# zkp-gravity/0g-halo2

Hardware: AMD Instinct MI355X
Metric: create_proof proofs/hour, model_28input_256entry_1hash_1bpi (higher is better)
Workload: dtype u32x8 (254-bit Montgomery integers)

## Files before the change

### 0g-halo2_amd/csrc/field.h

```cpp
#pragma once

#include <hip/hip_runtime.h>
#include <stdint.h>

#define ZG_HD __host__ __device__ __forceinline__

namespace zg {

struct alignas(16) Fe {
    uint32_t l[8];
};

struct FrParams {
    static ZG_HD uint32_t p(int i) {
        constexpr uint32_t P[8] = {0xf0000001u, 0x43e1f593u, 0x79b97091u, 0x2833e848u,
                                   0x8181585du, 0xb85045b6u, 0xe131a029u, 0x30644e72u};
        return P[i];
    }
    static constexpr uint32_t P_TOP = 0x30644e72u;
    static constexpr uint32_t INV = 0xefffffffu;
    static constexpr bool IS_FR = true;
    static ZG_HD Fe one() {
        return Fe{{0x4ffffffbu, 0xac96341cu, 0x9f60cd29u, 0x36fc7695u, 0x7879462eu, 0x666ea36fu,
                   0x9a07df2fu, 0x0e0a77c1u}};
// ... 122 lines not shown
    static ZG_HD Fe dbl(const Fe& a) { return add(a, a); }

    static ZG_HD Fe mul(const Fe& a, const Fe& b) {
#if defined(__HIP_DEVICE_COMPILE__)
        uint64_t acc = 0;
        uint32_t ovf = 0;
        uint32_t m[8], r[8];
#include "mont_mul_gfx950.inc"
        Fe o;
#pragma unroll
        for (int i = 0; i < 8; i++) o.l[i] = r[i];
        reduce_once(o);
        return o;
#else
        typedef unsigned __int128 u128;
        uint64_t A[4], B[4], M[4], t[6] = {0, 0, 0, 0, 0, 0};
        for (int i = 0; i < 4; i++) {
            A[i] = (uint64_t)a.l[2 * i] | ((uint64_t)a.l[2 * i + 1] << 32);
            B[i] = (uint64_t)b.l[2 * i] | ((uint64_t)b.l[2 * i + 1] << 32);
            M[i] = (uint64_t)P::p(2 * i) | ((uint64_t)P::p(2 * i + 1) << 32);
        }
        const uint64_t ninv32 = P::INV;
        const uint64_t inv64 = ninv32 * (2 + M[0] * ninv32);
        for (int i = 0; i < 4; i++) {
            u128 c = 0;
            for (int j = 0; j < 4; j++) {
                c += (u128)A[j] * B[i] + t[j];
                t[j] = (uint64_t)c;
                c >>= 64;
            }
            c += t[4];
            t[4] = (uint64_t)c;
            t[5] = (uint64_t)(c >> 64);
            const uint64_t m = t[0] * inv64;
            c = (u128)m * M[0] + t[0];
            c >>= 64;
            for (int j = 1; j < 4; j++) {
                c += (u128)m * M[j] + t[j];
                t[j - 1] = (uint64_t)c;
                c >>= 64;
            }
            c += t[4];
            t[3] = (uint64_t)c;
            t[4] = t[5] + (uint64_t)(c >> 64);
        }
        Fe o;
        for (int i = 0; i < 4; i++) {
            o.l[2 * i] = (uint32_t)t[i];
            o.l[2 * i + 1] = (uint32_t)(t[i] >> 32);
        }
        reduce_once(o);
        return o;
#endif
    }

    static ZG_HD Fe sqr(const Fe& a) { return mul(a, a); }

    static ZG_HD Fe from_raw(const Fe& a) { return mul(a, P::r2()); }

    static ZG_HD Fe to_raw(const Fe& a) {
        Fe one_raw = fe_zero();
        one_raw.l[0] = 1;
        return mul(a, one_raw);
    }

    static ZG_HD Fe from_u64(uint64_t v) {
        Fe t = fe_zero();
        t.l[0] = (uint32_t)v;
        t.l[1] = (uint32_t)(v >> 32);
        return from_raw(t);
    }

    static ZG_HD Fe pow(const Fe& a, const uint32_t e[8]) {
        Fe res = one();
        for (int i = 7; i >= 0; i--)
            for (int b = 31; b >= 0; b--) {
                res = sqr(res);
                if ((e[i] >> b) & 1) res = mul(res, a);
            }
        return res;
    }

    static ZG_HD Fe pow_u64(const Fe& a, uint64_t e) {
        Fe res = one();
        bool started = false;
        for (int b = 63; b >= 0; b--) {
            if (started) res = sqr(res);
            if ((e >> b) & 1) {
                res = mul(res, a);
                started = true;
            }
        }
        return res;
    }

    static ZG_HD Fe inv_fermat(const Fe& a) {
        uint32_t e[8];
#pragma unroll
        for (int i = 0; i < 8; i++) e[i] = P::p(i);
        e[0] -= 2;
        return pow(a, e);
    }

    static ZG_HD Fe inv(const Fe& a) {
        if (fe_is_zero(a)) return a;
#if !defined(__HIP_DEVICE_COMPILE__)
// ... 148 lines not shown
```

### 0g-halo2_amd/csrc/ntt.hip

```cpp
#include "poly.h"
#include "field9.h"

namespace zg {

struct NttArgs {
    const Fe* in;
    Fe* out;
    const Fe* tw;
    const Fe* tw_x;
    const Fe* tw_m;
    uint32_t tw_shift;
    size_t in_stride;
    size_t out_stride;
    uint32_t in_per, out_per;
    size_t in_outer, out_outer;
    uint32_t log_n, log_n1, log_n2;
    uint32_t in_len;
    uint32_t out_len;
    uint32_t coset_in;
    uint32_t coset_out;
    uint32_t scale_out;
    Fe zin0, zin1, zin2, zout0, zout1, zout2, scale;
};

__device__ __forceinline__ uint32_t bitrev(uint32_t v, uint32_t bits) {
    return bits == 0 ? 0u : (__brev(v) >> (32 - bits));
}

__device__ __forceinline__ Fe ld_fe(const Fe* p) {
    Fe r;
    const uint4* q = reinterpret_cast<const uint4*>(p);
    uint4 a = q[0], b = q[1];
    r.l[0] = a.x; r.l[1] = a.y; r.l[2] = a.z; r.l[3] = a.w;
    r.l[4] = b.x; r.l[5] = b.y; r.l[6] = b.z; r.l[7] = b.w;
    return r;
}

__device__ __forceinline__ void st_fe(Fe* p, const Fe& v) {
    uint4* q = reinterpret_cast<uint4*>(p);
    q[0] = make_uint4(v.l[0], v.l[1], v.l[2], v.l[3]);
    q[1] = make_uint4(v.l[4], v.l[5], v.l[6], v.l[7]);
}

template <int LOG_T, bool COLS, bool FIRST>
__global__ __launch_bounds__(1 << (LOG_T - 2)) void ntt_pass_kernel(NttArgs a) {
    constexpr uint32_t T = 1u << LOG_T;
    constexpr uint32_t NT = T / 4;
    extern __shared__ __align__(16) unsigned char smem[];
    uint4* XL = reinterpret_cast<uint4*>(smem);
    uint4* XH = XL + T;
    uint4* TL = XH + T;
    uint4* TH = TL + (1u << ((COLS ? a.log_n1 : a.log_n2) > 0 ? (COLS ? a.log_n1 : a.log_n2) - 1 : 0));
    auto slot = [](uint32_t i) { return i ^ ((i >> 3) & 7u) ^ ((i >> 6) & 7u) ^ ((i >> 9) & 7u); };
    auto ldx = [&](uint32_t i) {
        const uint32_t s = slot(i);
        const uint4 lo = XL[s], hi = XH[s];
        return Fe{{lo.x, lo.y, lo.z, lo.w, hi.x, hi.y, hi.z, hi.w}};
    };
    auto stx = [&](uint32_t i, const Fe& v) {
        const uint32_t s = slot(i);
        XL[s] = make_uint4(v.l[0], v.l[1], v.l[2], v.l[3]);
        XH[s] = make_uint4(v.l[4], v.l[5], v.l[6], v.l[7]);
    };
    auto ldt = [&](uint32_t i) {
        const uint32_t s = slot(i);
        const uint4 lo = TL[s], hi = TH[s];
        return Fe{{lo.x, lo.y, lo.z, lo.w, hi.x, hi.y, hi.z, hi.w}};
    };

    const uint32_t tid = threadIdx.x;
    const uint32_t log_m = COLS ? a.log_n1 : a.log_n2;
    const uint32_t M = 1u << log_m;
    const uint32_t N1 = 1u << a.log_n1, N2 = 1u << a.log_n2;
    uint32_t log_cnt = LOG_T - log_m;
    if (!COLS && log_cnt > a.log_n1) log_cnt = a.log_n1;
    const uint32_t cnt = 1u << log_cnt;
    const uint32_t tile = M << log_cnt;

    uint32_t nblk = gridDim.x, bid = blockIdx.x;
    if ((nblk & 7u) == 0) bid = (bid & 7u) * (nblk >> 3) + (bid >> 3);
    const uint32_t base = bid << log_cnt;

    const Fe* in = a.in + (size_t)(blockIdx.y / a.in_per) * a.in_outer + (size_t)(blockIdx.y % a.in_per) * a.in_stride;
    Fe* out = a.out + (size_t)(blockIdx.y / a.out_per) * a.out_outer + (size_t)(blockIdx.y % a.out_per) * a.out_stride;

    {
        const uint32_t tw_shift = a.log_n - log_m;
        for (uint32_t t = tid; t < M / 2; t += NT) {
            const Fe w = ld_fe(a.tw + ((size_t)t << tw_shift));
            const uint32_t s = slot(t);
            TL[s] = make_uint4(w.l[0], w.l[1], w.l[2], w.l[3]);
            TH[s] = make_uint4(w.l[4], w.l[5], w.l[6], w.l[7]);
        }
    }

    for (uint32_t e = tid; e < tile; e += NT) {
        uint32_t g, li;
        if (COLS) {
            uint32_t c = e & (cnt - 1), j1 = e >> log_cnt;
            g = j1 * N2 + base + c;
            li = e;
        } else {
            uint32_t j2 = e & (M - 1), r = e >> log_m;
            g = (base + r) * N2 + j2;
            li = e;
        }
        Fe v;
        if (FIRST) {
            if (g < a.in_len) {
                v = ld_fe(in + g);
                if (a.coset_in) {
                    const uint32_t m3 = g % 3u;
                    if (m3 != 0 || a.coset_in == 2) v = Fr::mul(v, m3 == 1 ? a.zin1 : m3 == 2 ? a.zin2 : a.zin0);
                }
            } else {
                v = fe_zero();
            }
        } else {
            v = ld_fe(in + g);
        }
        stx(li, v);
    }
    __syncthreads();

    auto at = [&](uint32_t sub, uint32_t e) { return COLS ? (e << log_cnt) + sub : (sub << log_m) + e; };
    uint32_t st = 0;
    if (FIRST && COLS && log_m >= 2) {
        const uint32_t nz_rows = (a.in_len + N2 - 1) >> a.log_n2;
        const uint32_t quarter = M >> 2, half = M >> 1;
        if (nz_rows <= quarter) {
            for (uint32_t g = tid; g < tile / 4; g += NT) {
                const uint32_t sub = g & (cnt - 1), i = g >> log_cnt;
                if (i >= nz_rows) continue;
                const uint32_t i0 = at(sub, i), i1 = at(sub, i + quarter), i2 = at(sub, i + half), i3 = at(sub, i + half + quarter);
                const Fe x0 = ldx(i0);
                Fe a2 = x0;
                if (i != 0) a2 = Fr::mul(x0, ldt(i));
                stx(i2, a2);
                if (i != 0) {
                    const Fe w = ldt(i << 1);
                    stx(i1, Fr::mul(x0, w));
                    stx(i3, Fr::mul(a2, w));
                } else {
                    stx(i1, x0);
                    stx(i3, a2);
                }
            }
            __syncthreads();
            st = 2;
        }
    }
    for (; st + 1 < log_m; st += 2) {
        const uint32_t log_half = log_m - st - 1, log_q = log_half - 1;
        const uint32_t half = 1u << log_half, quarter = 1u << log_q;
        for (uint32_t g = tid; g < tile / 4; g += NT) {
            uint32_t sub, b;
            if (COLS) {
                sub = g & (cnt - 1);
                b = g >> log_cnt;
            } else {
                b = g & (M / 4 - 1);
                sub = g >> (log_m - 2);
            }
            const uint32_t blk = b >> log_q, i = b & (quarter - 1);
            const uint32_t e0 = (blk << (log_half + 1)) + i;
            const uint32_t i0 = at(sub, e0), i1 = at(sub, e0 + quarter), i2 = at(sub, e0 + half), i3 = at(sub, e0 + half + quarter);
            const Fe x0 = ldx(i0), x1 = ldx(i1), x2 = ldx(i2), x3 = ldx(i3);
            const Fe a0 = Fr::add(x0, x2), a1 = Fr::add(x1, x3);
            Fe a2 = Fr::sub(x0, x2), a3 = Fr::sub(x1, x3);
            const uint32_t t0 = i << st;
            if (t0 != 0) a2 = Fr::mul(a2, ldt(t0));
            a3 = Fr::mul(a3, ldt((i + quarter) << st));
            const uint32_t t1 = i << (st + 1);
            stx(i0, Fr::add(a0, a1));
            stx(i2, Fr::add(a2, a3));
            Fe b1 = Fr::sub(a0, a1), b3 = Fr::sub(a2, a3);
            if (t1 != 0) {
                const Fe w = ldt(t1);
                b1 = Fr::mul(b1, w);
                b3 = Fr::mul(b3, w);
            }
            stx(i1, b1);
            stx(i3, b3);
        }
        __syncthreads();
    }
    const uint32_t nbf = tile / 2;
    for (; st < log_m; st++) {
        const uint32_t log_half = log_m - st - 1;
        const uint32_t half = 1u << log_half;
        for (uint32_t bf = tid; bf < nbf; bf += NT) {
            uint32_t s, b;
            if (COLS) {
                s = bf & (cnt - 1);
                b = bf >> log_cnt;
            } else {
                b = bf & (M / 2 - 1);
                s = bf >> (log_m - 1);
            }
            uint32_t blk = b >> log_half, i = b & (half - 1);
            uint32_t lo = (blk << (log_half + 1)) + i, hi = lo + half;
            uint32_t ilo = at(s, lo), ihi = at(s, hi);
            Fe u = ldx(ilo), v = ldx(ihi);
            stx(ilo, Fr::add(u, v));
            Fe d = Fr::sub(u, v);
            uint32_t twi = i << st;
            if (twi != 0) d = Fr::mul(d, ldt(twi));
            stx(ihi, d);
        }
        __syncthreads();
    }

    if (COLS) {
        for (uint32_t e = tid; e < tile; e += NT) {
            uint32_t c = e & (cnt - 1), pos = e >> log_cnt;
            uint32_t k1 = bitrev(pos, log_m);
            uint32_t j2 = base + c;
            Fe v = ldx(e);
            v = Fr::mul(v, ld_fe(a.tw_x + j2 * k1));
            st_fe(out + (size_t)k1 * N2 + j2, v);
        }
    } else {
        for (uint32_t e = tid; e < tile; e += NT) {
            uint32_t r = e & (cnt - 1), k2 = e >> log_cnt;
            uint32_t pos = bitrev(k2, log_m);
            uint32_t k = (base + r) + N1 * k2;
            if (k >= a.out_len) continue;
            Fe v = ldx((r << log_m) + pos);
            if (a.scale_out) v = Fr::mul(v, a.scale);
            if (a.coset_out) {
                const uint32_t m3 = k % 3u;
                if (m3 != 0 || a.coset_out == 2) v = Fr::mul(v, m3 == 1 ? a.zout1 : m3 == 2 ? a.zout2 : a.zout0);
            }
            st_fe(out + k, v);
        }
    }
}

template <int LOG_T, bool COLS, bool FIRST>
__global__ __launch_bounds__(1 << (LOG_T - 2)) void ntt9_pass_kernel(NttArgs a) {
    constexpr uint32_t T = 1u << LOG_T;
    constexpr uint32_t NT = T / 4;
    extern __shared__ __align__(16) unsigned char smem[];
    const uint32_t log_m = COLS ? a.log_n1 : a.log_n2;
    const uint32_t M = 1u << log_m;
    const uint32_t S = a.tw_shift;
    const uint32_t TWN = (M / 2) >> S ? (M / 2) >> S : 1;
    uint4* XL = reinterpret_cast<uint4*>(smem);
    uint4* XH = XL + T;
    uint4* TL = XH + T;
    uint4* TH = TL + TWN;
    int32_t* X8 = reinterpret_cast<int32_t*>(TH + TWN);
    int32_t* T8 = X8 + T;
    auto slot = [](uint32_t i) { return i ^ ((i >> 3) & 7u) ^ ((i >> 6) & 7u) ^ ((i >> 9) & 7u); };
    auto ld3 = [&](const uint4* L, const uint4* H, const int32_t* E, uint32_t i) {
        const uint32_t s = slot(i);
        const uint4 lo = L[s], hi = H[s];
        F9 r;
        r.l[0] = (int32_t)lo.x; r.l[1] = (int32_t)lo.y; r.l[2] = (int32_t)lo.z; r.l[3] = (int32_t)lo.w;
        r.l[4] = (int32_t)hi.x; r.l[5] = (int32_t)hi.y; r.l[6] = (int32_t)hi.z; r.l[7] = (int32_t)hi.w;
        r.l[8] = E[s];
        return r;
    };
    auto st3 = [&](uint4* L, uint4* H, int32_t* E, uint32_t i, const F9& v) {
        const uint32_t s = slot(i);
        L[s] = make_uint4((uint32_t)v.l[0], (uint32_t)v.l[1], (uint32_t)v.l[2], (uint32_t)v.l[3]);
        H[s] = make_uint4((uint32_t)v.l[4], (uint32_t)v.l[5], (uint32_t)v.l[6], (uint32_t)v.l[7]);
        E[s] = v.l[8];
    };
    auto ldx = [&](uint32_t i) { return ld3(XL, XH, X8, i); };
    auto stx = [&](uint32_t i, const F9& v) { st3(XL, XH, X8, i, v); };
    const Fe* twm9 = a.tw_m + M;
    auto ldt = [&](uint32_t i, uint32_t st) { return st >= S ? ld3(TL, TH, T8, i >> S) : f9_unpack(ld_fe(twm9 + i)); };

    const uint32_t tid = threadIdx.x;
    const uint32_t N1 = 1u << a.log_n1, N2 = 1u << a.log_n2;
    uint32_t log_cnt = LOG_T - log_m;
    if (!COLS && log_cnt > a.log_n1) log_cnt = a.log_n1;
    const uint32_t cnt = 1u << log_cnt;
    const uint32_t tile = M << log_cnt;

    uint32_t nblk = gridDim.x, bid = blockIdx.x;
    if ((nblk & 7u) == 0) bid = (bid & 7u) * (nblk >> 3) + (bid >> 3);
    const uint32_t base = bid << log_cnt;

    const Fe* in = a.in + (size_t)(blockIdx.y / a.in_per) * a.in_outer + (size_t)(blockIdx.y % a.in_per) * a.in_stride;
// ... 83 lines not shown
            if (reduce) s0 = Fr9::mul(s0, Fr9Params::one());
            stx(i0, s0);
            stx(i2, f9_norm(f9_add(a2, a3)));
            const F9 w = ldt(i << (st + 1), st + 1);
            stx(i1, Fr9::mul(f9_norm(f9_sub(a0, a1)), w));
            stx(i3, Fr9::mul(f9_sub(a2, a3), w));
        }
        __syncthreads();
    }
    const uint32_t nbf = tile / 2;
    for (; st < log_m; st++) {
        for (uint32_t bf = tid; bf < nbf; bf += NT) {
            uint32_t s, b;
            if (COLS) {
                s = bf & (cnt - 1);
                b = bf >> log_cnt;
            } else {
                b = bf & (M / 2 - 1);
                s = bf >> (log_m - 1);
            }
            const uint32_t ilo = at(s, b << 1), ihi = at(s, (b << 1) + 1);
            const F9 u = ldx(ilo), v = ldx(ihi);
            stx(ilo, f9_norm(f9_add(u, v)));
            stx(ihi, f9_norm(f9_sub(u, v)));
        }
        __syncthreads();
    }

    if (COLS) {
        for (uint32_t e = tid; e < tile; e += NT) {
            uint32_t c = e & (cnt - 1), pos = e >> log_cnt;
            uint32_t k1 = bitrev(pos, log_m);
            uint32_t j2 = base + c;
            const F9 v = Fr9::mul(ldx(e), f9_unpack(ld_fe(a.tw_x + j2 * k1)));
            st_fe(out + (size_t)k1 * N2 + j2, f9_reduce_pack<Fr9Params>(v));
        }
    } else {
        for (uint32_t e = tid; e < tile; e += NT) {
            uint32_t r = e & (cnt - 1), k2 = e >> log_cnt;
            uint32_t pos = bitrev(k2, log_m);
            uint32_t k = (base + r) + N1 * k2;
            if (k >= a.out_len) continue;
            F9 v = ldx((r << log_m) + pos);
            if (a.scale_out) v = Fr9::mul(v, f9_unpack(a.scale));
            if (a.coset_out) {
                const uint32_t m3 = k % 3u;
                if (m3 != 0 || a.coset_out == 2) v = Fr9::mul(v, f9_unpack(m3 == 1 ? a.zout1 : m3 == 2 ? a.zout2 : a.zout0));
            }
            st_fe(out + k, f9_reduce_pack<Fr9Params>(v));
        }
    }
}

__global__ void twiddle_kernel(Fe* tw, Fe omega, Fe s, uint32_t n) {
    constexpr uint32_t CH = 16;
    uint32_t i0 = (blockIdx.x * blockDim.x + threadIdx.x) * CH;
    if (i0 >= n) return;
    const Fe c261 = Fr9Params::c261_fe();
    Fe cur = Fr::mul(Fr::pow_u64(omega, i0), s);
    for (uint32_t j = 0; j < CH && i0 + j < n; j++) {
        st_fe(tw + i0 + j, cur);
        st_fe(tw + n + i0 + j, Fr::mul(cur, c261));
        cur = Fr::mul(cur, omega);
    }
}

constexpr uint32_t MAX_SCALED_TABLES = 8;
int get_twiddles(zg_ctx* ctx, uint32_t log_n, const Fe& omega, Fe** out, const Fe* scale) {
    const Fe s = scale ? *scale : Fr::one();
    TwiddleKey key;
    key.log_n = log_n;
    memcpy(key.omega.data(), &omega, 32);
    memcpy(key.scale.data(), &s, 32);
    DeviceState& ds = device_state(ctx->device);
    std::lock_guard<std::mutex> lock(ds.mu);
    auto it = ds.twiddles.find(key);
    if (it != ds.twiddles.end()) {
        *out = it->second;
        return ZG_OK;
    }
    if (scale) {
        const Fe one = Fr::one();
        uint32_t scaled = 0;
        for (const auto& kv : ds.twiddles) scaled += kv.first.log_n == log_n && memcmp(kv.first.scale.data(), &one, 32) != 0;
        if (scaled >= MAX_SCALED_TABLES) {
            *out = nullptr;
            return ZG_OK;
        }
    }
    uint32_t n = 1u << log_n;
    Fe* tw = nullptr;
    gate_yield(ctx);
    ZG_HIP(hipMalloc(&tw, (size_t)2 * n * sizeof(Fe)));
    uint32_t threads = 256, per = 16;
    uint32_t blocks = (n + threads * per - 1) / (threads * per);
    hipLaunchKernelGGL(twiddle_kernel, dim3(blocks), dim3(threads), 0, ctx->stream, tw, omega, s, n);
    hipError_t e = hipGetLastError();
    if (e == hipSuccess) e = hipStreamSynchronize(ctx->stream);
    if (e != hipSuccess) {
        (void)hipFree(tw);
        set_error("get_twiddles: %s", hipGetErrorString(e));
        return ZG_ERR_HIP;
    }
    ds.twiddles[key] = tw;
    *out = tw;
    return ZG_OK;
}

struct NttPlan {
    const Fe* in;
    size_t in_stride;
    Fe* out;
    size_t out_stride;
    size_t batch;
    uint32_t log_n;
    Fe omega;
    uint32_t in_len, out_len;
    Grouping grp;
    uint32_t coset_in = 0;
    uint32_t coset_out = 0;
    bool scale_out = false;
    bool hat = false;
    Fe zin0, zin1, zin2, zout0, zout1, zout2, scale;
};

static int sub_twiddles(zg_ctx* ctx, const NttPlan& p, uint32_t log_m, uint32_t log_t, const Fe** table, uint32_t* shift) {
    Fe om = p.omega;
    for (uint32_t i = log_m; i < p.log_n; i++) om = Fr::sqr(om);
    Fe* t = nullptr;
    ZG_TRY(get_twiddles(ctx, log_m, om, &t));
    *table = t;
    const uint32_t room = log_t == 10 ? 113u : 227u;
    uint32_t s = 0;
    while ((((1u << log_m) / 2) >> s) > room) s++;
    *shift = s;
    return ZG_OK;
}
static size_t nine_lds_bytes(uint32_t T, uint32_t log_m, uint32_t shift) {
    const uint32_t twn = ((1u << log_m) / 2) >> shift;
    return (size_t)(T + (twn ? twn : 1)) * 36;
}

template <int LOG_T, bool NINE>
static int launch_passes(zg_ctx* ctx, const NttPlan& p, const Fe* tw, const Fe* tw_x, Fe* tmp, size_t tmp_stride) {
    constexpr uint32_t T = 1u << LOG_T;
    constexpr size_t ELEM = NINE ? 36 : sizeof(Fe);
    NttArgs a;
    memset(&a, 0, sizeof(a));
    a.tw = tw;
    a.tw_x = tw_x;
    a.log_n = p.log_n;
    a.in_len = p.in_len;
    a.out_len = p.out_len;
    a.coset_in = p.coset_in;
    a.coset_out = p.coset_out;
    a.scale_out = p.scale_out;
    a.zin0 = p.zin0; a.zin1 = p.zin1; a.zin2 = p.zin2; a.zout0 = p.zout0; a.zout1 = p.zout1; a.zout2 = p.zout2; a.scale = p.scale;
    if (NINE) {
        const Fe c261 = Fr9Params::c261_fe();
        for (Fe* c : {&a.zin0, &a.zin1, &a.zin2, &a.zout0, &a.zout1, &a.zout2, &a.scale}) *c = Fr::mul(*c, c261);
    }
    const uint32_t N = 1u << p.log_n;
    const uint32_t gper = p.grp.per ? p.grp.per : 0xffffffffu;
    const double pass_bytes = (double)p.batch * ((double)p.in_len + (double)p.out_len) * 32.0;
    const double unit_bytes = ctx->unit_next >= 0.0 ? ctx->unit_next : pass_bytes;
    ctx->unit_next = -1.0;
    const double pts = (double)p.batch * (double)(1u << p.log_n) * 32.0;
    dim3 block(T / 4);
    const bool single = p.log_n <= (uint32_t)LOG_T;
    if (single) {
        a.log_n1 = 0;
        a.log_n2 = p.log_n;
        a.in = p.in; a.in_stride = p.in_stride;
        a.out = p.out; a.out_stride = p.out_stride;
        a.in_per = a.out_per = gper; a.in_outer = p.grp.in_outer; a.out_outer = p.grp.out_outer;
        size_t lds = (size_t)(T + (N > 1 ? N / 2 : 1)) * ELEM;
        if (NINE) {
            ZG_TRY(sub_twiddles(ctx, p, a.log_n2, LOG_T, &a.tw_m, &a.tw_shift));
            lds = nine_lds_bytes(T, a.log_n2, a.tw_shift);
        }
        if (NINE)
            ZG_LAUNCH_U(ctx, "ntt_single", pass_bytes, unit_bytes, (ntt9_pass_kernel<LOG_T, false, true>), dim3(1, (uint32_t)p.batch), block, lds, a);
        else
            ZG_LAUNCH_U(ctx, "ntt_single", pass_bytes, unit_bytes, (ntt_pass_kernel<LOG_T, false, true>), dim3(1, (uint32_t)p.batch), block, lds, a);
        ZG_HIP(hipGetLastError());
        return ZG_OK;
    }
    a.log_n1 = p.log_n / 2;
    a.log_n2 = p.log_n - a.log_n1;
    const uint32_t N1 = 1u << a.log_n1, N2 = 1u << a.log_n2;
    {
        a.in = p.in; a.in_stride = p.in_stride;
        a.out = tmp; a.out_stride = tmp_stride;
        a.in_per = gper; a.in_outer = p.grp.in_outer;
        a.out_per = 0xffffffffu; a.out_outer = 0;
        uint32_t cnt = T / N1;
        size_t lds = (size_t)(T + (N1 > 1 ? N1 / 2 : 1)) * ELEM;
        if (NINE) {
            ZG_TRY(sub_twiddles(ctx, p, a.log_n1, LOG_T, &a.tw_m, &a.tw_shift));
            lds = nine_lds_bytes(T, a.log_n1, a.tw_shift);
        }
        if (NINE)
            ZG_LAUNCH(ctx, "ntt_cols", (double)p.batch * (double)p.in_len * 32.0 + pts, (ntt9_pass_kernel<LOG_T, true, true>),
                      dim3(N2 / cnt, (uint32_t)p.batch), block, lds, a);
        else
            ZG_LAUNCH(ctx, "ntt_cols", (double)p.batch * (double)p.in_len * 32.0 + pts, (ntt_pass_kernel<LOG_T, true, true>),
                      dim3(N2 / cnt, (uint32_t)p.batch), block, lds, a);
        ZG_HIP(hipGetLastError());
    }
    {
        a.in = tmp; a.in_stride = tmp_stride;
        a.out = p.out; a.out_stride = p.out_stride;
        a.in_per = 0xffffffffu; a.in_outer = 0;
        a.out_per = gper; a.out_outer = p.grp.out_outer;
        uint32_t cnt = T / N2;
        if (cnt > N1) cnt = N1;
        size_t lds = (size_t)(T + (N2 > 1 ? N2 / 2 : 1)) * ELEM;
        if (NINE) {
            ZG_TRY(sub_twiddles(ctx, p, a.log_n2, LOG_T, &a.tw_m, &a.tw_shift));
            lds = nine_lds_bytes(T, a.log_n2, a.tw_shift);
        }
        if (NINE)
            ZG_LAUNCH_U(ctx, "ntt_rows", pts + (double)p.batch * (double)p.out_len * 32.0, unit_bytes, (ntt9_pass_kernel<LOG_T, false, false>),
                        dim3(N1 / cnt, (uint32_t)p.batch), block, lds, a);
        else
            ZG_LAUNCH_U(ctx, "ntt_rows", pts + (double)p.batch * (double)p.out_len * 32.0, unit_bytes, (ntt_pass_kernel<LOG_T, false, false>),
                        dim3(N1 / cnt, (uint32_t)p.batch), block, lds, a);
        ZG_HIP(hipGetLastError());
    }
    return ZG_OK;
}

static uint32_t ntt_log_t(uint32_t log_n) { return log_n <= 16 ? 10u : 11u; }
bool ntt_needs_tmp(uint32_t log_n) { return log_n > ntt_log_t(log_n); }

int ntt_run(zg_ctx* ctx, const NttPlan& plan, Fe* tmp, size_t tmp_stride) {
    ZG_REQUIRE(plan.log_n <= 22, ZG_ERR_UNSUPPORTED, "ntt: log_n %u > 22 not built", plan.log_n);
    if (plan.batch == 0) return ZG_OK;
    NttPlan p = plan;
    Fe* tw = nullptr;
    ZG_TRY(get_twiddles(ctx, p.log_n, p.omega, &tw));
    const int k9 = knob(K_NTT9);
    const bool nine = k9 < 0 ? ctx->msm_pair : k9 != 0;
    const Fe c32 = Fr::from_u64(32);
    const size_t half = (size_t)1 << p.log_n;
    const Fe c261 = Fr9Params::c261_fe();
    ZG_REQUIRE(memcmp(&c261, &c32, sizeof(Fe)) == 0, ZG_ERR_UNSUPPORTED, "ntt: 2^261 mod r is not the field element 32");
    const Fe* tw_x = tw + (nine ? half : 0);
    bool rides = false;
    if (ntt_needs_tmp(p.log_n) && (p.scale_out || p.hat)) {
        if (!nine && !p.scale_out) {
            tw_x = tw + half;
            rides = true;
        } else {
            Fe s = p.scale_out ? p.scale : Fr::one();
            if (p.hat) s = Fr::mul(s, c32);
            Fe* tws = nullptr;
            ZG_TRY(get_twiddles(ctx, p.log_n, p.omega, &tws, &s));
            if (tws) {
                tw_x = tws + (nine ? half : 0);
                rides = true;
            }
        }
    }
    if (rides) {
        p.scale_out = false;
    } else {
        if (p.hat) {
            ZG_REQUIRE(p.coset_in == 1, ZG_ERR_UNSUPPORTED, "ntt: a hat transform without coset constants");
            p.coset_in = 2;
// ... 251 lines not shown
```

Measured before the change: 5.508 million.

## Use Shoup-style precomputed-quotient twiddle multiplication and lazy reduction in NTT

Replaces Montgomery multiplication by twiddles in the non-nine NTT pass kernel with a Shoup-style constant multiply. Each twiddle is stored in raw form alongside a precomputed quotient floor(w*2^256/p), in a third table section. Butterflies use lazy add/sub in [0,2p) with a final reduce on output. This roughly doubles twiddle LDS footprint and per-twiddle LDS loads, adds hand-written gfx950 inline asm, and pins waves_per_eu to 5, trading some occupancy and LDS traffic for fewer multiply instructions.

```diff
diff --git a/0g-halo2_amd/csrc/field.h b/0g-halo2_amd/csrc/field.h
--- a/0g-halo2_amd/csrc/field.h
+++ b/0g-halo2_amd/csrc/field.h
@@ -198,6 +198,56 @@
         reduce_once(o);
         return o;
 #endif
+    }
+
+    static ZG_HD uint32_t negp(int i) { return i == 0 ? 0u - P::p(0) : ~P::p(i); }
+
+    static ZG_HD Fe mulc(const Fe& a, const Fe& w, const Fe& wq) {
+        uint32_t q[8], r[8];
+#if defined(__HIP_DEVICE_COMPILE__)
+        uint64_t acc;
+        uint32_t ovf;
+#include "mulc_gfx950.inc"
+#else
+        typedef unsigned __int128 u128;
+        u128 acc = 0;
+        for (int k = 6; k < 15; k++) {
+            for (int i = (k > 7 ? k - 7 : 0); i <= (k < 7 ? k : 7); i++) acc += (u128)((uint64_t)a.l[i] * wq.l[k - i]);
+            if (k >= 8) q[k - 8] = (uint32_t)acc;
+            acc >>= 32;
+        }
+        q[7] = (uint32_t)acc;
+        acc = 0;
+        for (int k = 0; k < 8; k++) {
+            for (int i = 0; i <= k; i++) acc += (u128)((uint64_t)a.l[i] * w.l[k - i]) + (u128)((uint64_t)q[i] * negp(k - i));
+            r[k] = (uint32_t)acc;
+            acc >>= 32;
+        }
+#endif
+        Fe o;
+#pragma unroll
+        for (int i = 0; i < 8; i++) o.l[i] = r[i];
+        return o;
+    }
+
+    static ZG_HD Fe mulc_quotient(const Fe& w) {
+        uint32_t pm[8], rem[8], t[8];
+        Fe q = fe_zero();
+#pragma unroll
+        for (int i = 0; i < 8; i++) {
+            pm[i] = P::p(i);
+            rem[i] = w.l[i];
+        }
+        for (int bit = 255; bit >= 0; bit--) {
+            add8(rem, rem, rem);
+            add8(q.l, q.l, q.l);
+            if (!sub8(t, rem, pm)) {
+#pragma unroll
+                for (int i = 0; i < 8; i++) rem[i] = t[i];
+                q.l[0] |= 1u;
+            }
+        }
+        return q;
     }
 
     static ZG_HD Fe sqr(const Fe& a) { return mul(a, a); }
diff --git a/0g-halo2_amd/csrc/mulc_gfx950.inc b/0g-halo2_amd/csrc/mulc_gfx950.inc
--- /dev/null
+++ b/0g-halo2_amd/csrc/mulc_gfx950.inc
@@ -0,0 +1,49 @@
+        asm("v_mad_u64_u32 %0, vcc, %2, %3, 0\n\tv_mov_b32 %1, 0\n\tv_mad_u64_u32 %0, vcc, %4, %5, %0\n\tv_addc_co_u32 %1, vcc, 0, %1, vcc\n\tv_mad_u64_u32 %0, vcc, %6, %7, %0\n\tv_addc_co_u32 %1, vcc, 0, %1, vcc\n\tv_mad_u64_u32 %0, vcc, %8, %9, %0\n\tv_addc_co_u32 %1, vcc, 0, %1, vcc\n\tv_mad_u64_u32 %0, vcc, %10, %11, %0\n\tv_addc_co_u32 %1, vcc, 0, %1, vcc\n\tv_mad_u64_u32 %0, vcc, %12, %13, %0\n\tv_addc_co_u32 %1, vcc, 0, %1, vcc\n\tv_mad_u64_u32 %0, vcc, %14, %15, %0\n\tv_addc_co_u32 %1, vcc, 0, %1, vcc" : "=&v"(acc), "=&v"(ovf) : "v"(a.l[0]), "v"(wq.l[6]), "v"(a.l[1]), "v"(wq.l[5]), "v"(a.l[2]), "v"(wq.l[4]), "v"(a.l[3]), "v"(wq.l[3]), "v"(a.l[4]), "v"(wq.l[2]), "v"(a.l[5]), "v"(wq.l[1]), "v"(a.l[6]), "v"(wq.l[0]) : "vcc");
+        acc = (acc >> 32) | ((uint64_t)ovf << 32);
+        asm("v_mad_u64_u32 %0, vcc, %2, %3, %0\n\tv_addc_co_u32 %1, vcc, 0, 0, vcc\n\tv_mad_u64_u32 %0, vcc, %4, %5, %0\n\tv_addc_co_u32 %1, vcc, 0, %1, vcc\n\tv_mad_u64_u32 %0, vcc, %6, %7, %0\n\tv_addc_co_u32 %1, vcc, 0, %1, vcc\n\tv_mad_u64_u32 %0, vcc, %8, %9, %0\n\tv_addc_co_u32 %1, vcc, 0, %1, vcc\n\tv_mad_u64_u32 %0, vcc, %10, %11, %0\n\tv_addc_co_u32 %1, vcc, 0, %1, vcc\n\tv_mad_u64_u32 %0, vcc, %12, %13, %0\n\tv_addc_co_u32 %1, vcc, 0, %1, vcc\n\tv_mad_u64_u32 %0, vcc, %14, %15, %0\n\tv_addc_co_u32 %1, vcc, 0, %1, vcc\n\tv_mad_u64_u32 %0, vcc, %16, %17, %0\n\tv_addc_co_u32 %1, vcc, 0, %1, vcc" : "+v"(acc), "=&v"(ovf) : "v"(a.l[0]), "v"(wq.l[7]), "v"(a.l[1]), "v"(wq.l[6]), "v"(a.l[2]), "v"(wq.l[5]), "v"(a.l[3]), "v"(wq.l[4]), "v"(a.l[4]), "v"(wq.l[3]), "v"(a.l[5]), "v"(wq.l[2]), "v"(a.l[6]), "v"(wq.l[1]), "v"(a.l[7]), "v"(wq.l[0]) : "vcc");
+        acc = (acc >> 32) | ((uint64_t)ovf << 32);
+        asm("v_mad_u64_u32 %0, vcc, %2, %3, %0\n\tv_addc_co_u32 %1, vcc, 0, 0, vcc\n\tv_mad_u64_u32 %0, vcc, %4, %5, %0\n\tv_addc_co_u32 %1, vcc, 0, %1, vcc\n\tv_mad_u64_u32 %0, vcc, %6, %7, %0\n\tv_addc_co_u32 %1, vcc, 0, %1, vcc\n\tv_mad_u64_u32 %0, vcc, %8, %9, %0\n\tv_addc_co_u32 %1, vcc, 0, %1, vcc\n\tv_mad_u64_u32 %0, vcc, %10, %11, %0\n\tv_addc_co_u32 %1, vcc, 0, %1, vcc\n\tv_mad_u64_u32 %0, vcc, %12, %13, %0\n\tv_addc_co_u32 %1, vcc, 0, %1, vcc\n\tv_mad_u64_u32 %0, vcc, %14, %15, %0\n\tv_addc_co_u32 %1, vcc, 0, %1, vcc" : "+v"(acc), "=&v"(ovf) : "v"(a.l[1]), "v"(wq.l[7]), "v"(a.l[2]), "v"(wq.l[6]), "v"(a.l[3]), "v"(wq.l[5]), "v"(a.l[4]), "v"(wq.l[4]), "v"(a.l[5]), "v"(wq.l[3]), "v"(a.l[6]), "v"(wq.l[2]), "v"(a.l[7]), "v"(wq.l[1]) : "vcc");
+        q[0] = (uint32_t)acc;
+        acc = (acc >> 32) | ((uint64_t)ovf << 32);
+        asm("v_mad_u64_u32 %0, vcc, %2, %3, %0\n\tv_addc_co_u32 %1, vcc, 0, 0, vcc\n\tv_mad_u64_u32 %0, vcc, %4, %5, %0\n\tv_addc_co_u32 %1, vcc, 0, %1, vcc\n\tv_mad_u64_u32 %0, vcc, %6, %7, %0\n\tv_addc_co_u32 %1, vcc, 0, %1, vcc\n\tv_mad_u64_u32 %0, vcc, %8, %9, %0\n\tv_addc_co_u32 %1, vcc, 0, %1, vcc\n\tv_mad_u64_u32 %0, vcc, %10, %11, %0\n\tv_addc_co_u32 %1, vcc, 0, %1, vcc\n\tv_mad_u64_u32 %0, vcc, %12, %13, %0\n\tv_addc_co_u32 %1, vcc, 0, %1, vcc" : "+v"(acc), "=&v"(ovf) : "v"(a.l[2]), "v"(wq.l[7]), "v"(a.l[3]), "v"(wq.l[6]), "v"(a.l[4]), "v"(wq.l[5]), "v"(a.l[5]), "v"(wq.l[4]), "v"(a.l[6]), "v"(wq.l[3]), "v"(a.l[7]), "v"(wq.l[2]) : "vcc");
+        q[1] = (uint32_t)acc;
+        acc = (acc >> 32) | ((uint64_t)ovf << 32);
+        asm("v_mad_u64_u32 %0, vcc, %2, %3, %0\n\tv_addc_co_u32 %1, vcc, 0, 0, vcc\n\tv_mad_u64_u32 %0, vcc, %4, %5, %0\n\tv_addc_co_u32 %1, vcc, 0, %1, vcc\n\tv_mad_u64_u32 %0, vcc, %6, %7, %0\n\tv_addc_co_u32 %1, vcc, 0, %1, vcc\n\tv_mad_u64_u32 %0, vcc, %8, %9, %0\n\tv_addc_co_u32 %1, vcc, 0, %1, vcc\n\tv_mad_u64_u32 %0, vcc, %10, %11, %0\n\tv_addc_co_u32 %1, vcc, 0, %1, vcc" : "+v"(acc), "=&v"(ovf) : "v"(a.l[3]), "v"(wq.l[7]), "v"(a.l[4]), "v"(wq.l[6]), "v"(a.l[5]), "v"(wq.l[5]), "v"(a.l[6]), "v"(wq.l[4]), "v"(a.l[7]), "v"(wq.l[3]) : "vcc");
+        q[2] = (uint32_t)acc;
+        acc = (acc >> 32) | ((uint64_t)ovf << 32);
+        asm("v_mad_u64_u32 %0, vcc, %2, %3, %0\n\tv_addc_co_u32 %1, vcc, 0, 0, vcc\n\tv_mad_u64_u32 %0, vcc, %4, %5, %0\n\tv_addc_co_u32 %1, vcc, 0, %1, vcc\n\tv_mad_u64_u32 %0, vcc, %6, %7, %0\n\tv_addc_co_u32 %1, vcc, 0, %1, vcc\n\tv_mad_u64_u32 %0, vcc, %8, %9, %0\n\tv_addc_co_u32 %1, vcc, 0, %1, vcc" : "+v"(acc), "=&v"(ovf) : "v"(a.l[4]), "v"(wq.l[7]), "v"(a.l[5]), "v"(wq.l[6]), "v"(a.l[6]), "v"(wq.l[5]), "v"(a.l[7]), "v"(wq.l[4]) : "vcc");
+        q[3] = (uint32_t)acc;
+        acc = (acc >> 32) | ((uint64_t)ovf << 32);
+        asm("v_mad_u64_u32 %0, vcc, %2, %3, %0\n\tv_addc_co_u32 %1, vcc, 0, 0, vcc\n\tv_mad_u64_u32 %0, vcc, %4, %5, %0\n\tv_addc_co_u32 %1, vcc, 0, %1, vcc\n\tv_mad_u64_u32 %0, vcc, %6, %7, %0\n\tv_addc_co_u32 %1, vcc, 0, %1, vcc" : "+v"(acc), "=&v"(ovf) : "v"(a.l[5]), "v"(wq.l[7]), "v"(a.l[6]), "v"(wq.l[6]), "v"(a.l[7]), "v"(wq.l[5]) : "vcc");
+        q[4] = (uint32_t)acc;
+        acc = (acc >> 32) | ((uint64_t)ovf << 32);
+        asm("v_mad_u64_u32 %0, vcc, %2, %3, %0\n\tv_addc_co_u32 %1, vcc, 0, 0, vcc\n\tv_mad_u64_u32 %0, vcc, %4, %5, %0\n\tv_addc_co_u32 %1, vcc, 0, %1, vcc" : "+v"(acc), "=&v"(ovf) : "v"(a.l[6]), "v"(wq.l[7]), "v"(a.l[7]), "v"(wq.l[6]) : "vcc");
+        q[5] = (uint32_t)acc;
+        acc = (acc >> 32) | ((uint64_t)ovf << 32);
+        asm("v_mad_u64_u32 %0, vcc, %2, %3, %0\n\tv_addc_co_u32 %1, vcc, 0, 0, vcc" : "+v"(acc), "=&v"(ovf) : "v"(a.l[7]), "v"(wq.l[7]) : "vcc");
+        q[6] = (uint32_t)acc;
+        acc = (acc >> 32) | ((uint64_t)ovf << 32);
+        q[7] = (uint32_t)acc;
+        asm("v_mad_u64_u32 %0, vcc, %2, %3, 0\n\tv_mov_b32 %1, 0\n\tv_mad_u64_u32 %0, vcc, %4, %5, %0\n\tv_addc_co_u32 %1, vcc, 0, %1, vcc" : "=&v"(acc), "=&v"(ovf) : "v"(a.l[0]), "v"(w.l[0]), "v"(q[0]), "s"(negp(0)) : "vcc");
+        r[0] = (uint32_t)acc;
+        acc = (acc >> 32) | ((uint64_t)ovf << 32);
+        asm("v_mad_u64_u32 %0, vcc, %2, %3, %0\n\tv_addc_co_u32 %1, vcc, 0, 0, vcc\n\tv_mad_u64_u32 %0, vcc, %4, %5, %0\n\tv_addc_co_u32 %1, vcc, 0, %1, vcc\n\tv_mad_u64_u32 %0, vcc, %6, %7, %0\n\tv_addc_co_u32 %1, vcc, 0, %1, vcc\n\tv_mad_u64_u32 %0, vcc, %8, %9, %0\n\tv_addc_co_u32 %1, vcc, 0, %1, vcc" : "+v"(acc), "=&v"(ovf) : "v"(a.l[0]), "v"(w.l[1]), "v"(a.l[1]), "v"(w.l[0]), "v"(q[0]), "s"(negp(1)), "v"(q[1]), "s"(negp(0)) : "vcc");
+        r[1] = (uint32_t)acc;
+        acc = (acc >> 32) | ((uint64_t)ovf << 32);
+        asm("v_mad_u64_u32 %0, vcc, %2, %3, %0\n\tv_addc_co_u32 %1, vcc, 0, 0, vcc\n\tv_mad_u64_u32 %0, vcc, %4, %5, %0\n\tv_addc_co_u32 %1, vcc, 0, %1, vcc\n\tv_mad_u64_u32 %0, vcc, %6, %7, %0\n\tv_addc_co_u32 %1, vcc, 0, %1, vcc\n\tv_mad_u64_u32 %0, vcc, %8, %9, %0\n\tv_addc_co_u32 %1, vcc, 0, %1, vcc\n\tv_mad_u64_u32 %0, vcc, %10, %11, %0\n\tv_addc_co_u32 %1, vcc, 0, %1, vcc\n\tv_mad_u64_u32 %0, vcc, %12, %13, %0\n\tv_addc_co_u32 %1, vcc, 0, %1, vcc" : "+v"(acc), "=&v"(ovf) : "v"(a.l[0]), "v"(w.l[2]), "v"(a.l[1]), "v"(w.l[1]), "v"(a.l[2]), "v"(w.l[0]), "v"(q[0]), "s"(negp(2)), "v"(q[1]), "s"(negp(1)), "v"(q[2]), "s"(negp(0)) : "vcc");
+        r[2] = (uint32_t)acc;
+        acc = (acc >> 32) | ((uint64_t)ovf << 32);
+        asm("v_mad_u64_u32 %0, vcc, %2, %3, %0\n\tv_addc_co_u32 %1, vcc, 0, 0, vcc\n\tv_mad_u64_u32 %0, vcc, %4, %5, %0\n\tv_addc_co_u32 %1, vcc, 0, %1, vcc\n\tv_mad_u64_u32 %0, vcc, %6, %7, %0\n\tv_addc_co_u32 %1, vcc, 0, %1, vcc\n\tv_mad_u64_u32 %0, vcc, %8, %9, %0\n\tv_addc_co_u32 %1, vcc, 0, %1, vcc\n\tv_mad_u64_u32 %0, vcc, %10, %11, %0\n\tv_addc_co_u32 %1, vcc, 0, %1, vcc\n\tv_mad_u64_u32 %0, vcc, %12, %13, %0\n\tv_addc_co_u32 %1, vcc, 0, %1, vcc\n\tv_mad_u64_u32 %0, vcc, %14, %15, %0\n\tv_addc_co_u32 %1, vcc, 0, %1, vcc\n\tv_mad_u64_u32 %0, vcc, %16, %17, %0\n\tv_addc_co_u32 %1, vcc, 0, %1, vcc" : "+v"(acc), "=&v"(ovf) : "v"(a.l[0]), "v"(w.l[3]), "v"(a.l[1]), "v"(w.l[2]), "v"(a.l[2]), "v"(w.l[1]), "v"(a.l[3]), "v"(w.l[0]), "v"(q[0]), "s"(negp(3)), "v"(q[1]), "s"(negp(2)), "v"(q[2]), "s"(negp(1)), "v"(q[3]), "s"(negp(0)) : "vcc");
+        r[3] = (uint32_t)acc;
+        acc = (acc >> 32) | ((uint64_t)ovf << 32);
+        asm("v_mad_u64_u32 %0, vcc, %2, %3, %0\n\tv_addc_co_u32 %1, vcc, 0, 0, vcc\n\tv_mad_u64_u32 %0, vcc, %4, %5, %0\n\tv_addc_co_u32 %1, vcc, 0, %1, vcc\n\tv_mad_u64_u32 %0, vcc, %6, %7, %0\n\tv_addc_co_u32 %1, vcc, 0, %1, vcc\n\tv_mad_u64_u32 %0, vcc, %8, %9, %0\n\tv_addc_co_u32 %1, vcc, 0, %1, vcc\n\tv_mad_u64_u32 %0, vcc, %10, %11, %0\n\tv_addc_co_u32 %1, vcc, 0, %1, vcc\n\tv_mad_u64_u32 %0, vcc, %12, %13, %0\n\tv_addc_co_u32 %1, vcc, 0, %1, vcc\n\tv_mad_u64_u32 %0, vcc, %14, %15, %0\n\tv_addc_co_u32 %1, vcc, 0, %1, vcc\n\tv_mad_u64_u32 %0, vcc, %16, %17, %0\n\tv_addc_co_u32 %1, vcc, 0, %1, vcc\n\tv_mad_u64_u32 %0, vcc, %18, %19, %0\n\tv_addc_co_u32 %1, vcc, 0, %1, vcc\n\tv_mad_u64_u32 %0, vcc, %20, %21, %0\n\tv_addc_co_u32 %1, vcc, 0, %1, vcc" : "+v"(acc), "=&v"(ovf) : "v"(a.l[0]), "v"(w.l[4]), "v"(a.l[1]), "v"(w.l[3]), "v"(a.l[2]), "v"(w.l[2]), "v"(a.l[3]), "v"(w.l[1]), "v"(a.l[4]), "v"(w.l[0]), "v"(q[0]), "s"(negp(4)), "v"(q[1]), "s"(negp(3)), "v"(q[2]), "s"(negp(2)), "v"(q[3]), "s"(negp(1)), "v"(q[4]), "s"(negp(0)) : "vcc");
+        r[4] = (uint32_t)acc;
+        acc = (acc >> 32) | ((uint64_t)ovf << 32);
+        asm("v_mad_u64_u32 %0, vcc, %2, %3, %0\n\tv_addc_co_u32 %1, vcc, 0, 0, vcc\n\tv_mad_u64_u32 %0, vcc, %4, %5, %0\n\tv_addc_co_u32 %1, vcc, 0, %1, vcc\n\tv_mad_u64_u32 %0, vcc, %6, %7, %0\n\tv_addc_co_u32 %1, vcc, 0, %1, vcc\n\tv_mad_u64_u32 %0, vcc, %8, %9, %0\n\tv_addc_co_u32 %1, vcc, 0, %1, vcc\n\tv_mad_u64_u32 %0, vcc, %10, %11, %0\n\tv_addc_co_u32 %1, vcc, 0, %1, vcc\n\tv_mad_u64_u32 %0, vcc, %12, %13, %0\n\tv_addc_co_u32 %1, vcc, 0, %1, vcc\n\tv_mad_u64_u32 %0, vcc, %14, %15, %0\n\tv_addc_co_u32 %1, vcc, 0, %1, vcc\n\tv_mad_u64_u32 %0, vcc, %16, %17, %0\n\tv_addc_co_u32 %1, vcc, 0, %1, vcc\n\tv_mad_u64_u32 %0, vcc, %18, %19, %0\n\tv_addc_co_u32 %1, vcc, 0, %1, vcc\n\tv_mad_u64_u32 %0, vcc, %20, %21, %0\n\tv_addc_co_u32 %1, vcc, 0, %1, vcc\n\tv_mad_u64_u32 %0, vcc, %22, %23, %0\n\tv_addc_co_u32 %1, vcc, 0, %1, vcc\n\tv_mad_u64_u32 %0, vcc, %24, %25, %0\n\tv_addc_co_u32 %1, vcc, 0, %1, vcc" : "+v"(acc), "=&v"(ovf) : "v"(a.l[0]), "v"(w.l[5]), "v"(a.l[1]), "v"(w.l[4]), "v"(a.l[2]), "v"(w.l[3]), "v"(a.l[3]), "v"(w.l[2]), "v"(a.l[4]), "v"(w.l[1]), "v"(a.l[5]), "v"(w.l[0]), "v"(q[0]), "s"(negp(5)), "v"(q[1]), "s"(negp(4)), "v"(q[2]), "s"(negp(3)), "v"(q[3]), "s"(negp(2)), "v"(q[4]), "s"(negp(1)), "v"(q[5]), "s"(negp(0)) : "vcc");
+        r[5] = (uint32_t)acc;
+        acc = (acc >> 32) | ((uint64_t)ovf << 32);
+        asm("v_mad_u64_u32 %0, vcc, %1, %2, %0\n\tv_mad_u64_u32 %0, vcc, %3, %4, %0\n\tv_mad_u64_u32 %0, vcc, %5, %6, %0\n\tv_mad_u64_u32 %0, vcc, %7, %8, %0\n\tv_mad_u64_u32 %0, vcc, %9, %10, %0\n\tv_mad_u64_u32 %0, vcc, %11, %12, %0\n\tv_mad_u64_u32 %0, vcc, %13, %14, %0\n\tv_mad_u64_u32 %0, vcc, %15, %16, %0\n\tv_mad_u64_u32 %0, vcc, %17, %18, %0\n\tv_mad_u64_u32 %0, vcc, %19, %20, %0\n\tv_mad_u64_u32 %0, vcc, %21, %22, %0\n\tv_mad_u64_u32 %0, vcc, %23, %24, %0\n\tv_mad_u64_u32 %0, vcc, %25, %26, %0\n\tv_mad_u64_u32 %0, vcc, %27, %28, %0" : "+v"(acc) : "v"(a.l[0]), "v"(w.l[6]), "v"(a.l[1]), "v"(w.l[5]), "v"(a.l[2]), "v"(w.l[4]), "v"(a.l[3]), "v"(w.l[3]), "v"(a.l[4]), "v"(w.l[2]), "v"(a.l[5]), "v"(w.l[1]), "v"(a.l[6]), "v"(w.l[0]), "v"(q[0]), "s"(negp(6)), "v"(q[1]), "s"(negp(5)), "v"(q[2]), "s"(negp(4)), "v"(q[3]), "s"(negp(3)), "v"(q[4]), "s"(negp(2)), "v"(q[5]), "s"(negp(1)), "v"(q[6]), "s"(negp(0)) : "vcc");
+        r[6] = (uint32_t)acc;
+        acc >>= 32;
+        asm("v_mad_u64_u32 %0, vcc, %1, %2, %0\n\tv_mad_u64_u32 %0, vcc, %3, %4, %0\n\tv_mad_u64_u32 %0, vcc, %5, %6, %0\n\tv_mad_u64_u32 %0, vcc, %7, %8, %0\n\tv_mad_u64_u32 %0, vcc, %9, %10, %0\n\tv_mad_u64_u32 %0, vcc, %11, %12, %0\n\tv_mad_u64_u32 %0, vcc, %13, %14, %0\n\tv_mad_u64_u32 %0, vcc, %15, %16, %0\n\tv_mad_u64_u32 %0, vcc, %17, %18, %0\n\tv_mad_u64_u32 %0, vcc, %19, %20, %0\n\tv_mad_u64_u32 %0, vcc, %21, %22, %0\n\tv_mad_u64_u32 %0, vcc, %23, %24, %0\n\tv_mad_u64_u32 %0, vcc, %25, %26, %0\n\tv_mad_u64_u32 %0, vcc, %27, %28, %0\n\tv_mad_u64_u32 %0, vcc, %29, %30, %0\n\tv_mad_u64_u32 %0, vcc, %31, %32, %0" : "+v"(acc) : "v"(a.l[0]), "v"(w.l[7]), "v"(a.l[1]), "v"(w.l[6]), "v"(a.l[2]), "v"(w.l[5]), "v"(a.l[3]), "v"(w.l[4]), "v"(a.l[4]), "v"(w.l[3]), "v"(a.l[5]), "v"(w.l[2]), "v"(a.l[6]), "v"(w.l[1]), "v"(a.l[7]), "v"(w.l[0]), "v"(q[0]), "s"(negp(7)), "v"(q[1]), "s"(negp(6)), "v"(q[2]), "s"(negp(5)), "v"(q[3]), "s"(negp(4)), "v"(q[4]), "s"(negp(3)), "v"(q[5]), "s"(negp(2)), "v"(q[6]), "s"(negp(1)), "v"(q[7]), "s"(negp(0)) : "vcc");
+        r[7] = (uint32_t)acc;
diff --git a/0g-halo2_amd/csrc/ntt.hip b/0g-halo2_amd/csrc/ntt.hip
--- a/0g-halo2_amd/csrc/ntt.hip
+++ b/0g-halo2_amd/csrc/ntt.hip
@@ -1,5 +1,6 @@
 #include "poly.h"
 #include "field9.h"
+#include "twiddle_table.h"
 
 namespace zg {
 
@@ -42,15 +43,51 @@
     q[1] = make_uint4(v.l[4], v.l[5], v.l[6], v.l[7]);
 }
 
+__device__ __forceinline__ uint32_t fr_2p(int i) { return (FrParams::p(i) << 1) | (i ? FrParams::p(i - 1) >> 31 : 0u); }
+
+__device__ __forceinline__ void lz_red(Fe& a) {
+    uint32_t pm[8], t[8];
+#pragma unroll
+    for (int i = 0; i < 8; i++) pm[i] = fr_2p(i);
+    if (!sub8(t, a.l, pm)) {
+#pragma unroll
+        for (int i = 0; i < 8; i++) a.l[i] = t[i];
+    }
+}
+
+__device__ __forceinline__ Fe lz_add(const Fe& a, const Fe& b) {
+    Fe o;
+    add8(o.l, a.l, b.l);
+    lz_red(o);
+    return o;
+}
+
+__device__ __forceinline__ Fe lz_sub(const Fe& a, const Fe& b) {
+    Fe o;
+    uint32_t pm[8];
+#pragma unroll
+    for (int i = 0; i < 8; i++) pm[i] = fr_2p(i);
+    sub8(o.l, a.l, b.l);
+    add8(o.l, o.l, pm);
+    return o;
+}
+
+struct TwC {
+    Fe w, q;
+};
+
 template <int LOG_T, bool COLS, bool FIRST>
-__global__ __launch_bounds__(1 << (LOG_T - 2)) void ntt_pass_kernel(NttArgs a) {
+__global__ __launch_bounds__(1 << (LOG_T - 2)) __attribute__((amdgpu_waves_per_eu(5, 5))) void ntt_pass_kernel(NttArgs a) {
     constexpr uint32_t T = 1u << LOG_T;
     constexpr uint32_t NT = T / 4;
     extern __shared__ __align__(16) unsigned char smem[];
     uint4* XL = reinterpret_cast<uint4*>(smem);
     uint4* XH = XL + T;
     uint4* TL = XH + T;
-    uint4* TH = TL + (1u << ((COLS ? a.log_n1 : a.log_n2) > 0 ? (COLS ? a.log_n1 : a.log_n2) - 1 : 0));
+    const uint32_t tslots = 1u << ((COLS ? a.log_n1 : a.log_n2) > 0 ? (COLS ? a.log_n1 : a.log_n2) - 1 : 0);
+    uint4* TH = TL + tslots;
+    uint4* QL = TH + tslots;
+    uint4* QH = QL + tslots;
     auto slot = [](uint32_t i) { return i ^ ((i >> 3) & 7u) ^ ((i >> 6) & 7u) ^ ((i >> 9) & 7u); };
     auto ldx = [&](uint32_t i) {
         const uint32_t s = slot(i);
@@ -64,9 +101,10 @@
     };
     auto ldt = [&](uint32_t i) {
         const uint32_t s = slot(i);
-        const uint4 lo = TL[s], hi = TH[s];
-        return Fe{{lo.x, lo.y, lo.z, lo.w, hi.x, hi.y, hi.z, hi.w}};
+        const uint4 lo = TL[s], hi = TH[s], qlo = QL[s], qhi = QH[s];
+        return TwC{Fe{{lo.x, lo.y, lo.z, lo.w, hi.x, hi.y, hi.z, hi.w}}, Fe{{qlo.x, qlo.y, qlo.z, qlo.w, qhi.x, qhi.y, qhi.z, qhi.w}}};
     };
+    auto mulc = [](const Fe& x, const TwC& t) { return Fr::mulc(x, t.w, t.q); };
 
     const uint32_t tid = threadIdx.x;
     const uint32_t log_m = COLS ? a.log_n1 : a.log_n2;
@@ -86,11 +124,15 @@
 
     {
         const uint32_t tw_shift = a.log_n - log_m;
+        const Fe* plain = a.tw + ((size_t)2 << a.log_n);
+        const Fe* quot = plain + ((size_t)1 << a.log_n >> 1);
         for (uint32_t t = tid; t < M / 2; t += NT) {
-            const Fe w = ld_fe(a.tw + ((size_t)t << tw_shift));
+            const Fe w = ld_fe(plain + ((size_t)t << tw_shift)), q = ld_fe(quot + ((size_t)t << tw_shift));
             const uint32_t s = slot(t);
             TL[s] = make_uint4(w.l[0], w.l[1], w.l[2], w.l[3]);
             TH[s] = make_uint4(w.l[4], w.l[5], w.l[6], w.l[7]);
+            QL[s] = make_uint4(q.l[0], q.l[1], q.l[2], q.l[3]);
+            QH[s] = make_uint4(q.l[4], q.l[5], q.l[6], q.l[7]);
         }
     }
 
@@ -135,12 +177,12 @@
                 const uint32_t i0 = at(sub, i), i1 = at(sub, i + quarter), i2 = at(sub, i + half), i3 = at(sub, i + half + quarter);
                 const Fe x0 = ldx(i0);
                 Fe a2 = x0;
-                if (i != 0) a2 = Fr::mul(x0, ldt(i));
+                if (i != 0) a2 = mulc(x0, ldt(i));
                 stx(i2, a2);
                 if (i != 0) {
-                    const Fe w = ldt(i << 1);
-                    stx(i1, Fr::mul(x0, w));
-                    stx(i3, Fr::mul(a2, w));
+                    const TwC w = ldt(i << 1);
+                    stx(i1, mulc(x0, w));
+                    stx(i3, mulc(a2, w));
                 } else {
                     stx(i1, x0);
                     stx(i3, a2);
@@ -166,19 +208,23 @@
             const uint32_t e0 = (blk << (log_half + 1)) + i;
             const uint32_t i0 = at(sub, e0), i1 = at(sub, e0 + quarter), i2 = at(sub, e0 + half), i3 = at(sub, e0 + half + quarter);
             const Fe x0 = ldx(i0), x1 = ldx(i1), x2 = ldx(i2), x3 = ldx(i3);
-            const Fe a0 = Fr::add(x0, x2), a1 = Fr::add(x1, x3);
-            Fe a2 = Fr::sub(x0, x2), a3 = Fr::sub(x1, x3);
+            const Fe a0 = lz_add(x0, x2), a1 = lz_add(x1, x3);
+            Fe a2 = lz_sub(x0, x2), a3 = lz_sub(x1, x3);
             const uint32_t t0 = i << st;
-            if (t0 != 0) a2 = Fr::mul(a2, ldt(t0));
-            a3 = Fr::mul(a3, ldt((i + quarter) << st));
+            if (t0 != 0) a2 = mulc(a2, ldt(t0));
+            else lz_red(a2);
+            a3 = mulc(a3, ldt((i + quarter) << st));
             const uint32_t t1 = i << (st + 1);
-            stx(i0, Fr::add(a0, a1));
-            stx(i2, Fr::add(a2, a3));
-            Fe b1 = Fr::sub(a0, a1), b3 = Fr::sub(a2, a3);
+            stx(i0, lz_add(a0, a1));
+            stx(i2, lz_add(a2, a3));
+            Fe b1 = lz_sub(a0, a1), b3 = lz_sub(a2, a3);
             if (t1 != 0) {
-                const Fe w = ldt(t1);
-                b1 = Fr::mul(b1, w);
-                b3 = Fr::mul(b3, w);
+                const TwC w = ldt(t1);
+                b1 = mulc(b1, w);
+                b3 = mulc(b3, w);
+            } else {
+                lz_red(b1);
+                lz_red(b3);
             }
             stx(i1, b1);
             stx(i3, b3);
@@ -202,10 +248,11 @@
             uint32_t lo = (blk << (log_half + 1)) + i, hi = lo + half;
             uint32_t ilo = at(s, lo), ihi = at(s, hi);
             Fe u = ldx(ilo), v = ldx(ihi);
-            stx(ilo, Fr::add(u, v));
-            Fe d = Fr::sub(u, v);
+            stx(ilo, lz_add(u, v));
+            Fe d = lz_sub(u, v);
             uint32_t twi = i << st;
-            if (twi != 0) d = Fr::mul(d, ldt(twi));
+            if (twi != 0) d = mulc(d, ldt(twi));
+            else lz_red(d);
             stx(ihi, d);
         }
         __syncthreads();
@@ -227,11 +274,19 @@
             uint32_t k = (base + r) + N1 * k2;
             if (k >= a.out_len) continue;
             Fe v = ldx((r << log_m) + pos);
-            if (a.scale_out) v = Fr::mul(v, a.scale);
+            bool canonical = log_m == 0;
+            if (a.scale_out) {
+                v = Fr::mul(v, a.scale);
+                canonical = true;
+            }
             if (a.coset_out) {
                 const uint32_t m3 = k % 3u;
-                if (m3 != 0 || a.coset_out == 2) v = Fr::mul(v, m3 == 1 ? a.zout1 : m3 == 2 ? a.zout2 : a.zout0);
-            }
+                if (m3 != 0 || a.coset_out == 2) {
+                    v = Fr::mul(v, m3 == 1 ? a.zout1 : m3 == 2 ? a.zout2 : a.zout0);
+                    canonical = true;
+                }
+            }
+            if (!canonical) Fr::reduce_once(v);
             st_fe(out + k, v);
         }
     }
@@ -421,18 +476,6 @@
     }
 }
 
-__global__ void twiddle_kernel(Fe* tw, Fe omega, Fe s, uint32_t n) {
-    constexpr uint32_t CH = 16;
-    uint32_t i0 = (blockIdx.x * blockDim.x + threadIdx.x) * CH;
-    if (i0 >= n) return;
-    const Fe c261 = Fr9Params::c261_fe();
-    Fe cur = Fr::mul(Fr::pow_u64(omega, i0), s);
-    for (uint32_t j = 0; j < CH && i0 + j < n; j++) {
-        st_fe(tw + i0 + j, cur);
-        st_fe(tw + n + i0 + j, Fr::mul(cur, c261));
-        cur = Fr::mul(cur, omega);
-    }
-}
 
 constexpr uint32_t MAX_SCALED_TABLES = 8;
 int get_twiddles(zg_ctx* ctx, uint32_t log_n, const Fe& omega, Fe** out, const Fe* scale) {
@@ -460,10 +503,8 @@
     uint32_t n = 1u << log_n;
     Fe* tw = nullptr;
     gate_yield(ctx);
-    ZG_HIP(hipMalloc(&tw, (size_t)2 * n * sizeof(Fe)));
-    uint32_t threads = 256, per = 16;
-    uint32_t blocks = (n + threads * per - 1) / (threads * per);
-    hipLaunchKernelGGL(twiddle_kernel, dim3(blocks), dim3(threads), 0, ctx->stream, tw, omega, s, n);
+    ZG_HIP(hipMalloc(&tw, twiddle_table_entries(n) * sizeof(Fe)));
+    launch_twiddle_table(ctx->stream, tw, omega, s, n);
     hipError_t e = hipGetLastError();
     if (e == hipSuccess) e = hipStreamSynchronize(ctx->stream);
     if (e != hipSuccess) {
@@ -514,6 +555,7 @@
 static int launch_passes(zg_ctx* ctx, const NttPlan& p, const Fe* tw, const Fe* tw_x, Fe* tmp, size_t tmp_stride) {
     constexpr uint32_t T = 1u << LOG_T;
     constexpr size_t ELEM = NINE ? 36 : sizeof(Fe);
+    constexpr size_t TWE = NINE ? 1 : 2;
     NttArgs a;
     memset(&a, 0, sizeof(a));
     a.tw = tw;
@@ -543,7 +585,7 @@
         a.in = p.in; a.in_stride = p.in_stride;
         a.out = p.out; a.out_stride = p.out_stride;
         a.in_per = a.out_per = gper; a.in_outer = p.grp.in_outer; a.out_outer = p.grp.out_outer;
-        size_t lds = (size_t)(T + (N > 1 ? N / 2 : 1)) * ELEM;
+        size_t lds = (size_t)(T + (N > 1 ? N / 2 : 1) * TWE) * ELEM;
         if (NINE) {
             ZG_TRY(sub_twiddles(ctx, p, a.log_n2, LOG_T, &a.tw_m, &a.tw_shift));
             lds = nine_lds_bytes(T, a.log_n2, a.tw_shift);
@@ -564,7 +606,7 @@
         a.in_per = gper; a.in_outer = p.grp.in_outer;
         a.out_per = 0xffffffffu; a.out_outer = 0;
         uint32_t cnt = T / N1;
-        size_t lds = (size_t)(T + (N1 > 1 ? N1 / 2 : 1)) * ELEM;
+        size_t lds = (size_t)(T + (N1 > 1 ? N1 / 2 : 1) * TWE) * ELEM;
         if (NINE) {
             ZG_TRY(sub_twiddles(ctx, p, a.log_n1, LOG_T, &a.tw_m, &a.tw_shift));
             lds = nine_lds_bytes(T, a.log_n1, a.tw_shift);
@@ -584,7 +626,7 @@
         a.out_per = gper; a.out_outer = p.grp.out_outer;
         uint32_t cnt = T / N2;
         if (cnt > N1) cnt = N1;
-        size_t lds = (size_t)(T + (N2 > 1 ? N2 / 2 : 1)) * ELEM;
+        size_t lds = (size_t)(T + (N2 > 1 ? N2 / 2 : 1) * TWE) * ELEM;
         if (NINE) {
             ZG_TRY(sub_twiddles(ctx, p, a.log_n2, LOG_T, &a.tw_m, &a.tw_shift));
             lds = nine_lds_bytes(T, a.log_n2, a.tw_shift);
diff --git a/0g-halo2_amd/csrc/twiddle_table.h b/0g-halo2_amd/csrc/twiddle_table.h
--- /dev/null
+++ b/0g-halo2_amd/csrc/twiddle_table.h
@@ -0,0 +1,44 @@
+#pragma once
+
+#include "field9.h"
+
+namespace zg {
+
+constexpr size_t twiddle_table_entries(uint32_t n) { return (size_t)3 * n; }
+
+__device__ __forceinline__ void tw_store(Fe* p, const Fe& v) {
+    uint4* q = reinterpret_cast<uint4*>(p);
+    q[0] = make_uint4(v.l[0], v.l[1], v.l[2], v.l[3]);
+    q[1] = make_uint4(v.l[4], v.l[5], v.l[6], v.l[7]);
+}
+
+__global__ void twiddle_kernel(Fe* tw, Fe omega, Fe s, uint32_t n) {
+    constexpr uint32_t CH = 16;
+    uint32_t i0 = (blockIdx.x * blockDim.x + threadIdx.x) * CH;
+    if (i0 >= n) return;
+    const Fe c261 = Fr9Params::c261_fe();
+    Fe cur = Fr::mul(Fr::pow_u64(omega, i0), s);
+    for (uint32_t j = 0; j < CH && i0 + j < n; j++) {
+        tw_store(tw + i0 + j, cur);
+        tw_store(tw + n + i0 + j, Fr::mul(cur, c261));
+        cur = Fr::mul(cur, omega);
+    }
+}
+
+__global__ void twiddle_quotient_kernel(Fe* tw, uint32_t n) {
+    const uint32_t i = blockIdx.x * blockDim.x + threadIdx.x;
+    if (i >= n / 2) return;
+    const uint4* q = reinterpret_cast<const uint4*>(tw + i);
+    const uint4 lo = q[0], hi = q[1];
+    const Fe w = Fr::to_raw(Fe{{lo.x, lo.y, lo.z, lo.w, hi.x, hi.y, hi.z, hi.w}});
+    tw_store(tw + (size_t)2 * n + i, w);
+    tw_store(tw + (size_t)2 * n + n / 2 + i, Fr::mulc_quotient(w));
+}
+
+inline void launch_twiddle_table(hipStream_t stream, Fe* tw, const Fe& omega, const Fe& s, uint32_t n) {
+    const uint32_t threads = 256, per = 16;
+    hipLaunchKernelGGL(twiddle_kernel, dim3((n + threads * per - 1) / (threads * per)), dim3(threads), 0, stream, tw, omega, s, n);
+    if (n >= 2) hipLaunchKernelGGL(twiddle_quotient_kernel, dim3((n / 2 + 63) / 64), dim3(64), 0, stream, tw, n);
+}
+
+}
```

Result: faster. 5.582 million (median of 6 runs) (+1.3%).
